# PaoloRibeca/KPop

Measured on AMD Instinct MI355X. Metric: sequences/sec end-to-end count->twist->distance, k=12, 100k x 150bp, higher is better.
Workload: dtype f64; 1 GPU; 100000 reads x 150 bp per GPU, k=12 DNA-ds, 65 class vectors, euclidean, metric powers(1,1,2); read_len=150, k=12, n_dims=64, n_classes=65, class_len=30000, twister=8390656 canonical k-mers x 64 dims, f64, synthetic, replicated on every GPU, reads_per_gpu=100000

## Files before the change

kpop_amd/csrc/class_set.hip:

```cpp
#include <algorithm>

#include "common.h"
#include "space_ops.h"
#include "distance_routes.h"

namespace kpop {

constexpr int kClassRows = 64;
constexpr int kClassGroup = 8;
constexpr int kClassFlight = 4;
constexpr uint32_t kClassSetMinRows = 128;

template <int KIND>
__global__ __launch_bounds__(256) void class_set_prepare_kernel(const double *__restrict__ m1, uint32_t r1, uint32_t n_dims, uint32_t dp,
                                                                const double *__restrict__ metric, double p, const double *__restrict__ norms1,
                                                                bool divide, double *__restrict__ n1_out, double *__restrict__ cls) {
  const uint32_t lane = threadIdx.x & 63u, i = blockIdx.x * 4u + (threadIdx.x >> 6);
  if (i >= r1) return;
  const bool in = lane < n_dims;
  const double el = in ? m1[(uint64_t)i * n_dims + lane] : 0.0, mc = in ? metric[lane] : 0.0;
  double nv = 1.0;
  if (divide) {
    if (norms1) {
      nv = norms1[i];
    } else {
      const double t = component<KIND>(el, mc, p);
      double acc = 0.0;
#pragma unroll
      for (int c = 0; c < 64; ++c)
        acc = __dadd_rn(acc, __hiloint2double(__builtin_amdgcn_readlane(__double2hiint(t), c), __builtin_amdgcn_readlane(__double2loint(t), c)));
      nv = scale_distance<KIND>(acc, p);
      nv = (nv == 0.0) ? 1.0 : nv;
      if (n1_out && lane == 0) n1_out[i] = nv;
    }
  }
  if (lane < dp) {
    cls[(uint64_t)i * 2u * dp + lane] = in ? (divide ? __ddiv_rn(el, nv) : el) : 0.0;
    cls[(uint64_t)i * 2u * dp + dp + lane] = mc;
  }
}

template <int KIND, int DP, int NC>
__device__ __forceinline__ void class_set_chain(const double (&x)[DP], const double *__restrict__ cls, uint32_t i, double p, double *stage) {
  double acc[NC];
#pragma unroll
  for (int k = 0; k < NC; ++k) acc[k] = 0.0;
  const double *__restrict__ a = cls + (uint64_t)i * (2 * DP);
  const double *__restrict__ metp = a + DP;
#pragma unroll
  for (int g = 0; g < DP; g += kClassGroup) {
#pragma unroll
    for (int d = 0; d < kClassGroup; ++d) {
      const double mc = metp[g + d];
#pragma unroll
      for (int k = 0; k < NC; ++k) {
        const double diff = __dsub_rn(a[k * (2 * DP) + g + d], x[g + d]);
        acc[k] = __dadd_rn(acc[k], component<KIND>(diff, mc, p));
      }
    }
  }
#pragma unroll
  for (int k = 0; k < NC; ++k) stage[i + k] = scale_distance<KIND>(acc[k], p);
}

template <int KIND, int DP, bool DIVIDE>
__global__ __launch_bounds__(256, DP == 64 ? 3 : 4) void class_set_distance_kernel(const double *__restrict__ cls,
                                                                                  uint32_t r1, const double *__restrict__ m2, uint32_t r2,
                                                                                  uint32_t n_dims, double p, double *__restrict__ n2,
                                                                                  double *__restrict__ out, uint32_t n_full, uint32_t tail_parts) {
  extern __shared__ __attribute__((aligned(16))) double class_lds[];
  constexpr int LD = DP + 1;
  constexpr int kPer = kClassRows * DP / 256;
  double *tile = class_lds;
  uint32_t rb = blockIdx.x, part = 0, parts = 1;
  if (blockIdx.x >= n_full) {
    const uint32_t t = blockIdx.x - n_full;
    rb = n_full + t / tail_parts;
    part = t % tail_parts;
    parts = tail_parts;
  }
  const uint32_t row0 = rb * (uint32_t)kClassRows;
  const uint32_t nrows = min((uint32_t)kClassRows, r2 - row0);
  {
    double pre[kPer];
#pragma unroll
    for (int u = 0; u < kPer; ++u) {
      const uint32_t e = threadIdx.x + 256u * u, i = e / DP, c = e % DP;
      pre[u] = m2[(uint64_t)min(row0 + i, r2 - 1u) * n_dims + min(c, n_dims - 1u)];
    }
#pragma unroll
    for (int u = 0; u < kPer; ++u) {
      const uint32_t e = threadIdx.x + 256u * u, i = e / DP, c = e % DP;
      tile[i * LD + c] = (i < nrows && c < n_dims) ? pre[u] : 0.0;
    }
  }
  __syncthreads();
  if (DIVIDE) {
    if (threadIdx.x < (uint32_t)kClassRows) {
      const double *row = tile + threadIdx.x * LD;
      const double *__restrict__ metp = cls + DP;
      double acc = 0.0;
#pragma unroll
      for (int c = 0; c < DP; ++c) acc = __dadd_rn(acc, component<KIND>(row[c], metp[c], p));
      double nv = scale_distance<KIND>(acc, p);
      nv = (nv == 0.0) ? 1.0 : nv;
      tile[threadIdx.x * LD + DP] = nv;
      if (threadIdx.x < nrows && part == 0) n2[row0 + threadIdx.x] = nv;
    }
    __syncthreads();
#pragma unroll
    for (int u = 0; u < kPer; ++u) {
      const uint32_t e = threadIdx.x + 256u * u, i = e / DP, c = e % DP;
      if (c < n_dims) tile[i * LD + c] = __ddiv_rn(tile[i * LD + c], tile[i * LD + DP]);
    }
    __syncthreads();
  }
  const uint32_t lane = threadIdx.x & 63u;
  double x[DP];
#pragma unroll
  for (int c = 0; c < DP; ++c) x[c] = tile[lane * LD + c];
  __syncthreads();
  const uint32_t wv = __builtin_amdgcn_readfirstlane(threadIdx.x >> 6);
  const uint32_t slices = 4u * parts, u = 4u * part + wv;
  const uint32_t c_hi = (u + 1u) * r1 / slices;
  const uint32_t RS = r1 | 1u;
  double *stage = class_lds + lane * RS;
  uint32_t i = u * r1 / slices;
  for (; i + kClassFlight <= c_hi; i += kClassFlight) class_set_chain<KIND, DP, kClassFlight>(x, cls, i, p, stage);
  for (; i < c_hi; ++i) class_set_chain<KIND, DP, 1>(x, cls, i, p, stage);
  __syncthreads();
  const uint32_t b_lo = part * r1 / parts, bw = (part + 1u) * r1 / parts - b_lo;
  if (bw == 0) return;
  const uint32_t total = nrows * bw, dj = 256u / bw, di = 256u % bw;
  double *__restrict__ dst = out + (uint64_t)row0 * r1 + b_lo;
  const double *src = class_lds + b_lo;
  uint32_t j = threadIdx.x / bw, ii = threadIdx.x % bw;
  for (uint32_t e = threadIdx.x; e < total; e += 256u) {
    dst[(uint64_t)j * r1 + ii] = src[j * RS + ii];
    j += dj;
    ii += di;
    if (ii >= bw) {
      ii -= bw;
      ++j;
    }
  }
}

static uint32_t class_set_padded_dims(uint32_t n_dims) { return n_dims <= 8 ? 8u : n_dims <= 16 ? 16u : n_dims <= 32 ? 32u : 64u; }

bool class_set_applies(int kind, uint32_t r1, uint32_t r2, uint32_t n_dims, uint64_t room_doubles) {
  const int mode = ctx().tune_class_set;
  if (mode == 0 || (kind != KPOP_EUCLIDEAN && kind != KPOP_COSINE)) return false;
  if (n_dims == 0 || n_dims > 64 || r1 < 1 || r1 >= 128 || r2 < 1 || r2 >= (1u << 30)) return false;
  const uint64_t dp = class_set_padded_dims(n_dims);
  if (2u * (uint64_t)r1 * dp > room_doubles) return false;
  return mode == 2 || r2 >= kClassSetMinRows;
}

template <int KIND, int DP>
static int launch_class_set_dp(const double *cls, uint32_t r1, const double *m2, uint32_t r2, uint32_t n_dims, double p,
                               bool divide, double *n2, double *out, hipStream_t st) {
  const uint32_t slots = (uint32_t)ctx().n_cus * (DP == 64 ? 3u : 4u), blocks = div_up(r2, kClassRows);
  const uint32_t tail = blocks % slots;
  uint32_t parts = 1;
  if (tail) parts = tail * 8u <= slots ? 8u : tail * 4u <= slots ? 4u : tail * 2u <= slots ? 2u : 1u;
  parts = std::max(1u, std::min(parts, r1 / 4u));
  const uint32_t n_full = parts > 1 ? blocks - tail : blocks;
  const dim3 grid(n_full + (blocks - n_full) * parts), block(256);
  const size_t lds = sizeof(double) * kClassRows * std::max<size_t>(DP + 1, r1 | 1u);
  if (divide) class_set_distance_kernel<KIND, DP, true><<<grid, block, lds, st>>>(cls, r1, m2, r2, n_dims, p, n2, out, n_full, parts);
  else class_set_distance_kernel<KIND, DP, false><<<grid, block, lds, st>>>(cls, r1, m2, r2, n_dims, p, n2, out, n_full, parts);
  KPOP_LAUNCH_CHECK();
  return 0;
}

template <int KIND>
static int launch_class_set_kind(const double *m1, uint32_t r1, const double *norms1, double *n1_out, const double *m2, uint32_t r2, double *n2,
                                 uint32_t n_dims, const double *metric, double p, bool divide, double *room, double *out, hipStream_t st) {
  const uint32_t dp = class_set_padded_dims(n_dims);
  double *cls = room;
  class_set_prepare_kernel<KIND><<<dim3(div_up(r1, 4)), dim3(256), 0, st>>>(m1, r1, n_dims, dp, metric, p, norms1, divide, n1_out, cls);
  KPOP_LAUNCH_CHECK();
  switch (dp) {
    case 8: return launch_class_set_dp<KIND, 8>(cls, r1, m2, r2, n_dims, p, divide, n2, out, st);
    case 16: return launch_class_set_dp<KIND, 16>(cls, r1, m2, r2, n_dims, p, divide, n2, out, st);
    case 32: return launch_class_set_dp<KIND, 32>(cls, r1, m2, r2, n_dims, p, divide, n2, out, st);
    default: return launch_class_set_dp<KIND, 64>(cls, r1, m2, r2, n_dims, p, divide, n2, out, st);
  }
}

int launch_class_set_distance(int kind, const double *m1, uint32_t r1, const double *norms1, double *n1_out, const double *m2, uint32_t r2, double *n2,
                              uint32_t n_dims, const double *metric, double p, bool divide, double *room, double *out, hipStream_t st) {
  if (kind == KPOP_EUCLIDEAN) return launch_class_set_kind<KPOP_EUCLIDEAN>(m1, r1, norms1, n1_out, m2, r2, n2, n_dims, metric, p, divide, room, out, st);
  return launch_class_set_kind<KPOP_COSINE>(m1, r1, norms1, n1_out, m2, r2, n2, n_dims, metric, p, divide, room, out, st);
}

}
```

Before: 78.06 million sequences/sec.

## Software-pipeline class-vector scalar loads in class-set distance kernel

Replaces compiler-scheduled reads of the class and metric vectors with explicit double-buffered s_load_dwordx8 scalar loads, issued one group ahead and waited on with lgkmcnt before compute. The flight width drops to 3 classes for DP>=32, and the tail is split into flights of 2 or 1. The prepare kernel now reduces the norm through LDS instead of 64 readlane pairs. The aim is to hide scalar-memory latency behind the f64 arithmetic in the distance loop. The inline asm relies on the compiler keeping the base address in SGPRs and is brittle about waitcnt correctness.

```diff
diff --git a/kpop_amd/csrc/class_set.hip b/kpop_amd/csrc/class_set.hip
--- a/kpop_amd/csrc/class_set.hip
+++ b/kpop_amd/csrc/class_set.hip
@@ -1,4 +1,5 @@
 #include <algorithm>
+#include <type_traits>
 
 #include "common.h"
 #include "space_ops.h"
@@ -7,28 +8,36 @@
 namespace kpop {
 
 constexpr int kClassRows = 64;
-constexpr int kClassGroup = 8;
-constexpr int kClassFlight = 4;
+template <int DP>
+struct ClassFlight {
+  static constexpr bool kPiped = DP >= 32;
+  static constexpr int kClasses = kPiped ? 3 : 4;
+};
 constexpr uint32_t kClassSetMinRows = 128;
 
 template <int KIND>
 __global__ __launch_bounds__(256) void class_set_prepare_kernel(const double *__restrict__ m1, uint32_t r1, uint32_t n_dims, uint32_t dp,
                                                                 const double *__restrict__ metric, double p, const double *__restrict__ norms1,
                                                                 bool divide, double *__restrict__ n1_out, double *__restrict__ cls) {
-  const uint32_t lane = threadIdx.x & 63u, i = blockIdx.x * 4u + (threadIdx.x >> 6);
-  if (i >= r1) return;
-  const bool in = lane < n_dims;
+  __shared__ __attribute__((aligned(16))) double terms[4][64];
+  const uint32_t lane = threadIdx.x & 63u, w = threadIdx.x >> 6, i = blockIdx.x * 4u + w;
+  const bool row = i < r1, in = row && lane < n_dims;
   const double el = in ? m1[(uint64_t)i * n_dims + lane] : 0.0, mc = in ? metric[lane] : 0.0;
+  const bool walk = divide && !norms1;
+  if (walk) terms[w][lane] = component<KIND>(el, mc, p);
+  __syncthreads();
+  if (!row) return;
   double nv = 1.0;
   if (divide) {
     if (norms1) {
       nv = norms1[i];
     } else {
-      const double t = component<KIND>(el, mc, p);
+      double t[64];
+#pragma unroll
+      for (int c = 0; c < 64; ++c) t[c] = terms[w][c];
       double acc = 0.0;
 #pragma unroll
-      for (int c = 0; c < 64; ++c)
-        acc = __dadd_rn(acc, __hiloint2double(__builtin_amdgcn_readlane(__double2hiint(t), c), __builtin_amdgcn_readlane(__double2loint(t), c)));
+      for (int c = 0; c < 64; ++c) acc = __dadd_rn(acc, t[c]);
       nv = scale_distance<KIND>(acc, p);
       nv = (nv == 0.0) ? 1.0 : nv;
       if (n1_out && lane == 0) n1_out[i] = nv;
@@ -41,26 +50,95 @@
 }
 
 template <int KIND, int DP, int NC>
-__device__ __forceinline__ void class_set_chain(const double (&x)[DP], const double *__restrict__ cls, uint32_t i, double p, double *stage) {
+__device__ __forceinline__ void class_set_flight(const double (&x)[DP], const double *__restrict__ cls, uint32_t i, double p, double *stage) {
   double acc[NC];
 #pragma unroll
   for (int k = 0; k < NC; ++k) acc[k] = 0.0;
   const double *__restrict__ a = cls + (uint64_t)i * (2 * DP);
   const double *__restrict__ metp = a + DP;
 #pragma unroll
-  for (int g = 0; g < DP; g += kClassGroup) {
-#pragma unroll
-    for (int d = 0; d < kClassGroup; ++d) {
-      const double mc = metp[g + d];
+  for (int d = 0; d < DP; ++d) {
+    const double mc = metp[d];
+#pragma unroll
+    for (int k = 0; k < NC; ++k) {
+      const double diff = __dsub_rn(a[k * (2 * DP) + d], x[d]);
+      acc[k] = __dadd_rn(acc[k], component<KIND>(diff, mc, p));
+    }
+  }
+#pragma unroll
+  for (int k = 0; k < NC; ++k) stage[i + k] = scale_distance<KIND>(acc[k], p);
+}
+
+template <int I, int N, class F>
+__device__ __forceinline__ void class_static_for(F &&f) {
+  if constexpr (I < N) {
+    f(std::integral_constant<int, I>{});
+    class_static_for<I + 1, N>(f);
+  }
+}
+
+typedef uint32_t class_quad __attribute__((ext_vector_type(8)));
+
+template <int BYTES>
+__device__ __forceinline__ void class_quad_load(class_quad &q, const double *base) {
+  asm volatile("s_load_dwordx8 %0, %1, %2" : "=s"(q) : "s"(base), "i"(BYTES));
+}
+
+template <int NC>
+__device__ __forceinline__ void class_quads_arrived(class_quad (&q)[NC + 1]) {
+  asm volatile("s_waitcnt lgkmcnt(0)" : "+s"(q[0]));
+#pragma unroll
+  for (int k = 1; k <= NC; ++k) asm volatile("" : "+s"(q[k]));
+}
+
+__device__ __forceinline__ double class_quad_at(const class_quad &q, int d) { return __hiloint2double((int)q[2 * d + 1], (int)q[2 * d]); }
+
+template <int KIND, int DP, int NC>
+__device__ __forceinline__ void class_set_flight_piped(const double (&x)[DP], const double *__restrict__ cls, uint32_t i, double p, double *stage) {
+  constexpr int G = 4, NG = DP / G;
+  double acc[NC];
+#pragma unroll
+  for (int k = 0; k < NC; ++k) acc[k] = 0.0;
+  const double *__restrict__ a = cls + (uint64_t)i * (2 * DP);
+  class_quad q[2][NC + 1];
+  auto issue = [&](auto g_) {
+    constexpr int g = decltype(g_)::value;
+    class_static_for<0, NC>([&](auto k_) {
+      constexpr int k = decltype(k_)::value;
+      class_quad_load<(k * 2 * DP + g * G) * 8>(q[g & 1][k], a);
+    });
+    class_quad_load<(DP + g * G) * 8>(q[g & 1][NC], a);
+  };
+  auto group = [&](auto g_) {
+    constexpr int g = decltype(g_)::value;
+    class_quads_arrived<NC>(q[g & 1]);
+    if constexpr (g + 1 < NG) issue(std::integral_constant<int, g + 1>{});
+    __builtin_amdgcn_sched_barrier(0);
+#pragma unroll
+    for (int d = 0; d < G; ++d) {
+      const double mc = class_quad_at(q[g & 1][NC], d);
 #pragma unroll
       for (int k = 0; k < NC; ++k) {
-        const double diff = __dsub_rn(a[k * (2 * DP) + g + d], x[g + d]);
+        const double diff = __dsub_rn(class_quad_at(q[g & 1][k], d), x[g * G + d]);
         acc[k] = __dadd_rn(acc[k], component<KIND>(diff, mc, p));
       }
     }
-  }
+  };
+  issue(std::integral_constant<int, 0>{});
+  class_static_for<0, NG>(group);
 #pragma unroll
   for (int k = 0; k < NC; ++k) stage[i + k] = scale_distance<KIND>(acc[k], p);
+}
+
+template <int KIND, int DP, int N, int LO>
+__device__ __forceinline__ void class_set_flight_of(const double (&x)[DP], const double *__restrict__ cls, uint32_t i, uint32_t n, double p,
+                                                    double *stage) {
+  if (N == LO || n == (uint32_t)N) {
+    if constexpr (ClassFlight<DP>::kPiped) class_set_flight_piped<KIND, DP, N>(x, cls, i, p, stage);
+    else class_set_flight<KIND, DP, N>(x, cls, i, p, stage);
+  } else if constexpr (N > LO) {
+    class_set_flight_of<KIND, DP, N - 1, LO>(x, cls, i, n, p, stage);
+  }
 }
 
 template <int KIND, int DP, bool DIVIDE>
@@ -120,14 +198,21 @@
 #pragma unroll
   for (int c = 0; c < DP; ++c) x[c] = tile[lane * LD + c];
   __syncthreads();
+  constexpr int NC = ClassFlight<DP>::kClasses;
   const uint32_t wv = __builtin_amdgcn_readfirstlane(threadIdx.x >> 6);
   const uint32_t slices = 4u * parts, u = 4u * part + wv;
   const uint32_t c_hi = (u + 1u) * r1 / slices;
   const uint32_t RS = r1 | 1u;
   double *stage = class_lds + lane * RS;
   uint32_t i = u * r1 / slices;
-  for (; i + kClassFlight <= c_hi; i += kClassFlight) class_set_chain<KIND, DP, kClassFlight>(x, cls, i, p, stage);
-  for (; i < c_hi; ++i) class_set_chain<KIND, DP, 1>(x, cls, i, p, stage);
+  uint32_t left = c_hi - i;
+  for (; left >= (uint32_t)NC && left != (uint32_t)NC + 1u; i += NC, left -= NC) class_set_flight_of<KIND, DP, NC, NC>(x, cls, i, NC, p, stage);
+  while (left != 0u) {
+    const uint32_t n = left > (uint32_t)NC - 1u ? 2u : left;
+    class_set_flight_of<KIND, DP, NC - 1, 1>(x, cls, i, n, p, stage);
+    i += n;
+    left -= n;
+  }
   __syncthreads();
   const uint32_t b_lo = part * r1 / parts, bw = (part + 1u) * r1 / parts - b_lo;
   if (bw == 0) return;
```

Measured after the change: 78.28 million sequences/sec (median of 6 runs). About the same (+0.3%).

## Software-pipeline class-vector scalar loads with inline asm in class-set distance

Applied to the files above, without the earlier changes.

Replaces the compiler-scheduled loop over class rows with hand-issued s_load_dwordx4/x8 scalar loads. The next group of class and metric values is fetched while the current group is computed, and an explicit lgkmcnt wait plus sched barriers enforce the overlap. The tail handling switches from a scalar loop to a single chain of width 1 to 3. This targets scalar memory latency stalls in the distance inner loop. The cost is fragile inline asm that assumes a diff*diff*m component, which static_asserts enforce for euclidean/cosine only, and the possibility of higher SGPR pressure.

```diff
diff --git a/kpop_amd/csrc/class_set.hip b/kpop_amd/csrc/class_set.hip
--- a/kpop_amd/csrc/class_set.hip
+++ b/kpop_amd/csrc/class_set.hip
@@ -7,9 +7,9 @@
 namespace kpop {
 
 constexpr int kClassRows = 64;
-constexpr int kClassGroup = 8;
 constexpr int kClassFlight = 4;
 constexpr uint32_t kClassSetMinRows = 128;
+constexpr int class_set_group(int dp) { return dp == 8 ? 2 : 4; }
 
 template <int KIND>
 __global__ __launch_bounds__(256) void class_set_prepare_kernel(const double *__restrict__ m1, uint32_t r1, uint32_t n_dims, uint32_t dp,
@@ -40,25 +40,97 @@
   }
 }
 
+template <int NC, int W>
+struct ClassOperands {
+  typedef double row __attribute__((ext_vector_type(W)));
+  row a[NC], m;
+};
+
+#define KPOP_CLASS_SET_ISSUE(LOAD)                                                                                                         \
+  if constexpr (NC == 1)                                                                                                                   \
+    asm volatile(LOAD " %0, %2, %3\n\t" LOAD " %1, %2, %4" : "=&s"(o.m), "=&s"(o.a[0]) : "s"(a), "n"(kMet), "n"(kAt));                   \
+  else if constexpr (NC == 2)                                                                                                              \
+    asm volatile(LOAD " %0, %3, %4\n\t" LOAD " %1, %3, %5\n\t" LOAD " %2, %3, %6"                                                        \
+                 : "=&s"(o.m), "=&s"(o.a[0]), "=&s"(o.a[1])                                                                                \
+                 : "s"(a), "n"(kMet), "n"(kAt), "n"(kRow + kAt));                                                                          \
+  else if constexpr (NC == 3)                                                                                                              \
+    asm volatile(LOAD " %0, %4, %5\n\t" LOAD " %1, %4, %6\n\t" LOAD " %2, %4, %7\n\t" LOAD " %3, %4, %8"                                \
+                 : "=&s"(o.m), "=&s"(o.a[0]), "=&s"(o.a[1]), "=&s"(o.a[2])                                                                 \
+                 : "s"(a), "n"(kMet), "n"(kAt), "n"(kRow + kAt), "n"(2 * kRow + kAt));                                                     \
+  else                                                                                                                                     \
+    asm volatile(LOAD " %0, %5, %6\n\t" LOAD " %1, %5, %7\n\t" LOAD " %2, %5, %8\n\t" LOAD " %3, %5, %9\n\t" LOAD " %4, %5, %10"        \
+                 : "=&s"(o.m), "=&s"(o.a[0]), "=&s"(o.a[1]), "=&s"(o.a[2]), "=&s"(o.a[3])                                                  \
+                 : "s"(a), "n"(kMet), "n"(kAt), "n"(kRow + kAt), "n"(2 * kRow + kAt), "n"(3 * kRow + kAt))
+
+template <int DP, int NC, int W, int G>
+__device__ __forceinline__ void class_set_issue(ClassOperands<NC, W> &o, const double *a) {
+  constexpr int kRow = 2 * DP * 8, kAt = G * 8, kMet = DP * 8 + G * 8;
+  static_assert(NC >= 1 && NC <= 4 && (W == 2 || W == 4) && 3 * kRow + kMet < (1 << 20), "the offsets are immediates of 21 signed bits");
+  if constexpr (W == 4) {
+    KPOP_CLASS_SET_ISSUE("s_load_dwordx8");
+  } else {
+    KPOP_CLASS_SET_ISSUE("s_load_dwordx4");
+  }
+}
+#undef KPOP_CLASS_SET_ISSUE
+
+template <int NC, int W>
+__device__ __forceinline__ void class_set_land(ClassOperands<NC, W> &o, double (&acc)[NC]) {
+  if constexpr (NC == 1) asm volatile("s_waitcnt lgkmcnt(0)" : "+s"(o.m), "+s"(o.a[0]), "+v"(acc[0]));
+  else if constexpr (NC == 2) asm volatile("s_waitcnt lgkmcnt(0)" : "+s"(o.m), "+s"(o.a[0]), "+s"(o.a[1]), "+v"(acc[0]), "+v"(acc[1]));
+  else if constexpr (NC == 3)
+    asm volatile("s_waitcnt lgkmcnt(0)" : "+s"(o.m), "+s"(o.a[0]), "+s"(o.a[1]), "+s"(o.a[2]), "+v"(acc[0]), "+v"(acc[1]), "+v"(acc[2]));
+  else
+    asm volatile("s_waitcnt lgkmcnt(0)"
+                 : "+s"(o.m), "+s"(o.a[0]), "+s"(o.a[1]), "+s"(o.a[2]), "+s"(o.a[3]), "+v"(acc[0]), "+v"(acc[1]), "+v"(acc[2]), "+v"(acc[3]));
+}
+
+template <int KIND, int DP, int NC, int W, int G>
+__device__ __forceinline__ void class_set_groups(const double (&x)[DP], const double *a, const ClassOperands<NC, W> &cur, double (&acc)[NC]) {
+  static_assert(KIND == KPOP_EUCLIDEAN || KIND == KPOP_COSINE, "the component is diff *. diff *. m");
+  constexpr bool kMore = G + W < DP;
+  ClassOperands<NC, W> nxt;
+  if constexpr (kMore) class_set_issue<DP, NC, W, G + W>(nxt, a);
+  __builtin_amdgcn_sched_barrier(0);
+  constexpr int kDims = NC >= 3 ? 1 : NC == 2 ? 2 : W;
+#pragma unroll
+  for (int d0 = 0; d0 < W; d0 += kDims) {
+    double t[kDims][NC];
+#pragma unroll
+    for (int d = 0; d < kDims; ++d)
+#pragma unroll
+      for (int k = 0; k < NC; ++k) t[d][k] = __dsub_rn(cur.a[k][d0 + d], x[G + d0 + d]);
+#pragma unroll
+    for (int d = 0; d < kDims; ++d)
+#pragma unroll
+      for (int k = 0; k < NC; ++k) t[d][k] = __dmul_rn(t[d][k], t[d][k]);
+#pragma unroll
+    for (int d = 0; d < kDims; ++d)
+#pragma unroll
+      for (int k = 0; k < NC; ++k) t[d][k] = __dmul_rn(t[d][k], cur.m[d0 + d]);
+#pragma unroll
+    for (int d = 0; d < kDims; ++d)
+#pragma unroll
+      for (int k = 0; k < NC; ++k) acc[k] = __dadd_rn(acc[k], t[d][k]);
+  }
+  __builtin_amdgcn_sched_barrier(0);
+  if constexpr (kMore) {
+    class_set_land<NC, W>(nxt, acc);
+    class_set_groups<KIND, DP, NC, W, G + W>(x, a, nxt, acc);
+  }
+}
+
 template <int KIND, int DP, int NC>
 __device__ __forceinline__ void class_set_chain(const double (&x)[DP], const double *__restrict__ cls, uint32_t i, double p, double *stage) {
+  constexpr int W = class_set_group(DP);
   double acc[NC];
 #pragma unroll
   for (int k = 0; k < NC; ++k) acc[k] = 0.0;
-  const double *__restrict__ a = cls + (uint64_t)i * (2 * DP);
-  const double *__restrict__ metp = a + DP;
-#pragma unroll
-  for (int g = 0; g < DP; g += kClassGroup) {
-#pragma unroll
-    for (int d = 0; d < kClassGroup; ++d) {
-      const double mc = metp[g + d];
-#pragma unroll
-      for (int k = 0; k < NC; ++k) {
-        const double diff = __dsub_rn(a[k * (2 * DP) + g + d], x[g + d]);
-        acc[k] = __dadd_rn(acc[k], component<KIND>(diff, mc, p));
-      }
-    }
-  }
+  const double *a = cls + (uint64_t)i * (2 * DP);
+  ClassOperands<NC, W> first;
+  class_set_issue<DP, NC, W, 0>(first, a);
+  class_set_land<NC, W>(first, acc);
+  class_set_groups<KIND, DP, NC, W, 0>(x, a, first, acc);
 #pragma unroll
   for (int k = 0; k < NC; ++k) stage[i + k] = scale_distance<KIND>(acc[k], p);
 }
@@ -127,7 +199,12 @@
   double *stage = class_lds + lane * RS;
   uint32_t i = u * r1 / slices;
   for (; i + kClassFlight <= c_hi; i += kClassFlight) class_set_chain<KIND, DP, kClassFlight>(x, cls, i, p, stage);
-  for (; i < c_hi; ++i) class_set_chain<KIND, DP, 1>(x, cls, i, p, stage);
+  switch (c_hi - i) {
+    case 3: class_set_chain<KIND, DP, 3>(x, cls, i, p, stage); break;
+    case 2: class_set_chain<KIND, DP, 2>(x, cls, i, p, stage); break;
+    case 1: class_set_chain<KIND, DP, 1>(x, cls, i, p, stage); break;
+    default: break;
+  }
   __syncthreads();
   const uint32_t b_lo = part * r1 / parts, bw = (part + 1u) * r1 / parts - b_lo;
   if (bw == 0) return;
```

Measured after the change: 78.18 million sequences/sec before, 78.35 million sequences/sec after (median of 6 runs). No clear change (+0.2%).
